# UbiquitousLearning/Mandheling-DSP-Training

Hardware: AMD Instinct MI355X
Metric: training images/sec + int8 MFMA TOPS, VGG-11 batch 256, 1/2/4/8 MI355X (higher is better)
Workload: dtype int8; 1 GPU; VGG11 NITI int8 training step (fwd+relu+pool, loss grad, weight grad, input grad, SGD), 3x32x32; global_batch=256, per_gpu_batch=256, parallelism=single GPU, streams=one stream (weight gradient, then input gradient, per layer)

## Files before the change

### include/niti_hip.h

```cpp
#ifndef NITI_HIP_H
#define NITI_HIP_H

#include <stddef.h>
#include <stdint.h>

#ifdef __cplusplus
extern "C" {
#endif

enum niti_error_code {
    NITI_NO_ERROR = 0,
    NITI_OUT_OF_MEMORY = 1,
    NITI_NOT_SUPPORT = 2,
    NITI_COMPUTE_SIZE_ERROR = 3,
    NITI_NO_EXECUTION = 4,
    NITI_INVALID_VALUE = 5,
    NITI_INPUT_DATA_ERROR = 10,
    NITI_CALL_BACK_STOP = 11
};

enum niti_op_type {
    NITI_OP_CONV_INT8 = 700,
    NITI_OP_DECONV_INT8 = 701,
    NITI_OP_RELU_INT8 = 703,
// ... 158 lines not shown
    int8_t* pool3_out;
    int8_t* pool3_arg;
    int relu, pool_relu, pool_h, pool_w;
    int zero_cls, zc_h, zc_w;
    int pool3_h, pool3_w, pool3_oh, pool3_ow;
} niti_requant_fused;
int niti_requant_act_fused(const int32_t* acc, int64_t rows, int ldc, const uint32_t* amax,
                           const niti_requant_fused* f, void* stream);
int niti_requant_grad(const int32_t* acc, int64_t n, const uint32_t* amax, int rule, int8_t* g_out,
                      int8_t* w_update, void* stream);
int niti_sgd_update(const int32_t* acc, const uint32_t* amax, int rule, int co, int ci, int kk, int cip, int cop,
                    int8_t* w_ohwi16, int8_t* wt_ihwo16, int8_t* g_out, void* stream);
int niti_sgd_update_wf(const int32_t* acc, const uint32_t* amax, int rule, int co, int ci, int kk, int cip, int cop,
                       int8_t* w_ohwi16, int8_t* wt_ihwo16, int8_t* g_out, int8_t* wf, int8_t* wft, void* stream);
typedef struct niti_sgd_combine_job {
    const int32_t* slab;
    int splits;
    int64_t stride;
    int64_t n;
    int32_t* acc;
    uint32_t* amax;
} niti_sgd_combine_job;
int niti_sgd_combine(const niti_sgd_combine_job* jobs, int n_jobs, void* stream);
int niti_nhwc16_to_chwn16(const int8_t* in, int n, int hw, int cp, int np, int8_t* out, void* stream);
int niti_ohwi16_to_ihwo16(const int8_t* w, int co, int ci, int kk, int cip, int cop, int8_t* wt, void* stream);
int niti_nchw_to_nhwc16(const int8_t* x, int n, int c, int hw, int cp, int8_t* out, void* stream);
int niti_nchw_to_chwn16(const int8_t* x, int n, int c, int hw, int cp, int np, int8_t* out, void* stream);
int niti_nhwc16_to_nchw(const int8_t* x, int n, int c, int hw, int cp, int8_t* out, void* stream);
int niti_oihw_to_ohwi16(const int8_t* w, int co, int ci, int kk, int cip, int8_t* out, void* stream);
int niti_ohwi16_to_oihw(const int8_t* w, int co, int ci, int kk, int cip, int8_t* out, void* stream);
int niti_residual_add(const int8_t* a, const int8_t* ea, const int8_t* b, const int8_t* eb, int64_t n, int32_t* z,
                      int8_t* ez, uint32_t* amax, void* stream);
int niti_residual_requant(const int8_t* a, const int8_t* ea, const int8_t* b, const int8_t* eb, int64_t n,
                          const uint32_t* amax, int8_t* ez, int8_t* exp_out, int relu, int8_t* out, void* stream);
int niti_residual_requant_relu_grad(const int8_t* a, const int8_t* ea, const int8_t* b, const int8_t* eb, int64_t n,
                                    const uint32_t* amax, int8_t* ez, int8_t* exp_out, const int8_t* relu_mask,
                                    int8_t* out, void* stream);
int niti_sum_pool(const int8_t* x, int n, int hw, int cp, int32_t* acc, uint32_t* amax, void* stream);
int niti_sum_pool_grad(const int8_t* dy, int n, int hw, int cp, int8_t* dx, void* stream);
int niti_im2col(const niti_geom* g, const int8_t* x, int kp, int8_t* xcol, void* stream);
int niti_im2col_nchw(const niti_geom* g, const int8_t* x_nchw, int kp, int8_t* xcol, void* stream);
int niti_maxpool(const int8_t* x, int n, int h, int w, int cp, int k, int s, int p, int8_t* y, int oh, int ow,
                 void* stream);
int niti_maxpool_grad(const int8_t* x, const int8_t* y, const int8_t* dy, int n, int h, int w, int cp, int k,
                      int s, int p, int oh, int ow, int relu, int8_t* dx, void* stream);
int niti_maxpool_grad_ws(const int8_t* x, const int8_t* y, const int8_t* dy, int n, int h, int w, int cp, int k,
// ... 113 lines not shown
```

### mandheling-dsp-training_amd/csrc/niti_capi.hip

```cpp
#include "../../include/niti_hip.h"
#include <memory>
#include <vector>

#include "niti_internal.hpp"
#include "niti_kernels.hpp"

struct niti_execution {
    niti::Execution* impl = nullptr;
    int op = 0;
    std::vector<void*> stage;
    std::vector<size_t> stage_bytes;
    uint32_t* err_host = nullptr;
    ~niti_execution() {
        delete impl;
        for (void* p : stage)
            if (p) (void)hipFree(p);
        if (err_host) (void)hipHostFree(err_host);
    }
};

namespace {
int code(hipError_t e) {
    if (e == hipSuccess) return NITI_NO_ERROR;
    if (e == hipErrorOutOfMemory) return NITI_OUT_OF_MEMORY;
// ... 588 lines not shown
    j.wft = wft;
    return code(niti::sgd_update_many(&j, 1, S(stream)));
}

int niti_sgd_combine(const niti_sgd_combine_job* jobs, int n_jobs, void* stream) {
    if (!jobs || n_jobs < 1 || n_jobs > niti::SGD_MAX_JOBS) return NITI_INVALID_VALUE;
    niti::SgdJob r[niti::SGD_MAX_JOBS];
    for (int j = 0; j < n_jobs; ++j) {
        const niti_sgd_combine_job& s = jobs[j];
        if (!s.slab || !s.acc || !s.amax || s.splits < 1 || s.n < 4 || s.n % 4 || s.stride % 4 || s.stride < s.n)
            return NITI_INVALID_VALUE;
        if (((uintptr_t)s.slab | (uintptr_t)s.acc) & 15) return NITI_INVALID_VALUE;
        r[j] = niti::SgdJob{};
        r[j].acc = s.acc;
        r[j].amax = s.amax;
        r[j].slab = s.slab;
        r[j].splits = s.splits;
        r[j].slab_stride = s.stride;
        r[j].slab_n = s.n;
    }
    return code(niti::sgd_combine_many(r, n_jobs, S(stream)));
}

int niti_nhwc16_to_chwn16(const int8_t* in, int n, int hw, int cp, int np, int8_t* out, void* stream) {
    return code(niti::nhwc16_to_chwn16(in, n, hw, cp, np, out, S(stream)));
}
int niti_ohwi16_to_ihwo16(const int8_t* w, int co, int ci, int kk, int cip, int cop, int8_t* wt, void* stream) {
    return code(niti::ohwi16_to_ihwo16(w, co, ci, kk, cip, cop, wt, S(stream)));
}
int niti_nchw_to_nhwc16(const int8_t* x, int n, int c, int hw, int cp, int8_t* out, void* stream) {
    return code(niti::nchw_to_nhwc16(x, n, c, hw, cp, out, S(stream)));
}
int niti_nchw_to_chwn16(const int8_t* x, int n, int c, int hw, int cp, int np, int8_t* out, void* stream) {
    return code(niti::nchw_to_chwn16(x, n, c, hw, cp, np, out, S(stream)));
}
int niti_nhwc16_to_nchw(const int8_t* x, int n, int c, int hw, int cp, int8_t* out, void* stream) {
    return code(niti::nhwc16_to_nchw(x, n, c, hw, cp, out, S(stream)));
}
int niti_oihw_to_ohwi16(const int8_t* w, int co, int ci, int kk, int cip, int8_t* out, void* stream) {
    return code(niti::oihw_to_ohwi16(w, co, ci, kk, cip, out, S(stream)));
}
int niti_ohwi16_to_oihw(const int8_t* w, int co, int ci, int kk, int cip, int8_t* out, void* stream) {
    return code(niti::ohwi16_to_oihw(w, co, ci, kk, cip, out, S(stream)));
}
int niti_residual_add(const int8_t* a, const int8_t* ea, const int8_t* b, const int8_t* eb, int64_t n, int32_t* z,
                      int8_t* ez, uint32_t* amax, void* stream) {
// ... 207 lines not shown
```

### mandheling-dsp-training_amd/csrc/niti_device.hpp

```cpp
#pragma once

#include <hip/hip_runtime.h>
#include <stdint.h>

#include "niti_kernels.hpp"

namespace niti {

typedef int v2i __attribute__((ext_vector_type(2)));
typedef int v4i __attribute__((ext_vector_type(4)));
typedef int v16i __attribute__((ext_vector_type(16)));
typedef signed char v16c __attribute__((ext_vector_type(16)));

constexpr uint32_t OOB = 0x80000000u;

__device__ __forceinline__ __amdgpu_buffer_rsrc_t make_rsrc(const void* p, uint32_t bytes) {
    return __builtin_amdgcn_make_buffer_rsrc((void*)p, (short)0, (int)bytes, 0x00020000);
}
__device__ __forceinline__ v4i buf_load16(__amdgpu_buffer_rsrc_t r, uint32_t off) {
    return __builtin_bit_cast(v4i, __builtin_amdgcn_raw_buffer_load_b128(r, (int)off, 0, 0));
}

struct FastDiv {
    uint32_t m = 1, s = 0, d = 1;
};
static inline FastDiv make_fastdiv(uint32_t d) {
    FastDiv f;
    f.d = d;
    f.s = 0;
    while ((1ull << f.s) < d) ++f.s;
    f.m = (uint32_t)((((uint64_t)1 << 32) * ((1ull << f.s) - d)) / d + 1);
    return f;
}
__device__ __forceinline__ uint32_t fdiv(const FastDiv& f, uint32_t n) { return (__umulhi(n, f.m) + n) >> f.s; }

__device__ __forceinline__ uint32_t uabs32(int v) { return v < 0 ? 0u - (uint32_t)v : (uint32_t)v; }

__device__ __forceinline__ uint32_t wave_max(uint32_t v) {
#pragma unroll
    for (int o = 32; o > 0; o >>= 1) {
        const uint32_t t = __shfl_xor(v, o, 64);
        v = v > t ? v : t;
    }
// ... 276 lines not shown
```

### mandheling-dsp-training_amd/csrc/niti_kernels.hip

```cpp
#include <stdlib.h>

#include <map>
#include <atomic>
#include <mutex>
#include <type_traits>
#include <vector>
#include <algorithm>
#include <stdio.h>

#include <hip/hip_ext.h>

#include "niti_device.hpp"
#include "niti_gridbar.hpp"
#include "niti_kernels.hpp"
#include "niti_sgd.hpp"
#include "niti_map.hpp"

namespace niti {


bool ConvGeom::finalize() {
    if (n <= 0 || c_in <= 0 || h <= 0 || w <= 0 || c_out <= 0 || kh <= 0 || kw <= 0) return false;
    if (sh <= 0 || sw <= 0 || dh <= 0 || dw <= 0) return false;
    const int keh = dh * (kh - 1) + 1, kew = dw * (kw - 1) + 1;
// ... 3188 lines not shown
    int64_t blocks = (n16 + 255) / 256;
    blocks = blocks < 1 ? 1 : blocks > 2048 ? 2048 : blocks;
    static const int pk = getenv("NITI_RES_PK") ? atoi(getenv("NITI_RES_PK")) : 1;
    hipLaunchKernelGGL(residual_requant_kernel, dim3((unsigned)blocks), dim3(256), 0, st, a, ea, b, eb, n16, amax, ez,
                       exp_out, relu, relu_mask, out, spec, slot, pk);
    return hipGetLastError();
}

struct Conv0 {
    const int8_t* x;
    const int8_t* w;
    uint32_t wbytes;
    int co, cop, oh, ow;
    int64_t units;
    uint32_t* amax;
    int8_t* out;
    int8_t* pool_out;
    int8_t* pool_c32;
    int8_t* out_c32;
    int8_t* pool_code;
    const int8_t *exp_in, *wscale;
    int8_t* exp_out;
    int relu;
};

template <int PASS>
__global__ void __launch_bounds__(256) conv0_kernel(Conv0 g) {
    const int lane = threadIdx.x & 63;
    const int wave = blockIdx.x * 4 + (threadIdx.x >> 6), nwaves = gridDim.x * 4;
    const int h = lane >> 5, c = lane & 31;
    const __amdgpu_buffer_rsrc_t rw = make_rsrc(g.w, g.wbytes);
    int s = 2, shift = 0;
    bool raw = false;
    if (PASS == 1) {
        const int bw = bitwidth_of(read_max(g.amax));
        shift = bw - 7;
        s = shift > 1 ? shift : 2;
        raw = shift <= 0;
        if (blockIdx.x == 0 && threadIdx.x == 0 && g.exp_out != nullptr) {
            const int inc = shift > 1 ? shift : (shift == 1 ? 2 : 0);
            *g.exp_out = (int8_t)((g.exp_in ? (int)*g.exp_in : 0) + (g.wscale ? (int)*g.wscale : 0) + inc);
        }
    }
    const int tiles = g.cop / 32;
    uint32_t m = 0;
    const int segs = g.ow / 32, pairs = g.oh / 2;
    for (int64_t u = wave; u < g.units; u += nwaves) {
        const int seg = (int)(u % segs);
        const int64_t rest = u / segs;
        const int pr = (int)(rest % pairs);
        const int64_t img = rest / pairs;
        const int64_t p0 = (img * g.oh + 2 * pr) * g.ow + seg * 32;
        v4i a[2];
#pragma unroll
        for (int r = 0; r < 2; ++r) a[r] = *(const v4i*)(g.x + (p0 + (int64_t)r * g.ow + c) * 32 + 16 * h);
        for (int t = 0; t < tiles; ++t) {
            const v4i b = buf_load16(rw, (uint32_t)((t * 32 + c) * 32 + 16 * h));
            v16i acc[2];
// ... 69 lines not shown
                        }
                    }
                    if ((c & 1) == 0) {
                        const int64_t pp = (img * (g.oh / 2) + pr) * (g.ow / 2) + seg * 16 + (c >> 1);
                        *(v4i*)(g.pool_out + pp * g.cop + t * 32 + 16 * h) = v;
                        if (g.pool_code != nullptr) *(v4i*)(g.pool_code + pp * g.cop + t * 32 + 16 * h) = code;
                        if (g.pool_c32 != nullptr) {
                            const int64_t hw2 = (int64_t)(g.oh / 2) * (g.ow / 2);
                            *(v4i*)(g.pool_c32 + ((img * tiles + t) * hw2 + pp - img * hw2) * 32 + 16 * h) = v;
                        }
                    }
                }
            }
        }
    }
    if (PASS == 0) {
        m = wave_max(m);
        __shared__ uint32_t red[4];
        if (lane == 0) red[threadIdx.x >> 6] = m;
        __syncthreads();
        if (threadIdx.x == 0) publish_max(g.amax, max(max(red[0], red[1]), max(red[2], red[3])));
    }
}

bool conv0_ok(const ConvGeom& g) {
    return g.kh == 1 && g.kw == 1 && g.c_in == 32 && g.cip == 32 && g.ow % 32 == 0 && g.oh % 2 == 0 && g.sh == 1 &&
           g.pt == 0 && g.cop % 32 == 0;
}

hipError_t conv0_fwd(const ConvGeom& g, const int8_t* xcol, const int8_t* w, uint32_t* amax, const ActOut& o,
                     int pass, hipStream_t st, int8_t* pool_c32, int8_t* out_c32, int8_t* pool_code) {
    if (!conv0_ok(g) || o.relu_mask != nullptr) return hipErrorInvalidValue;
    if (o.out == nullptr && (pass == 1 && (o.pool.pool_out == nullptr || pool_code == nullptr))) return hipErrorInvalidValue;
    if ((pool_c32 != nullptr || pool_code != nullptr) && o.pool.pool_out == nullptr) return hipErrorInvalidValue;
    Conv0 k{};
    k.x = xcol;
    k.w = w;
    k.wbytes = (uint32_t)((int64_t)g.c_out * 32);
    k.co = g.c_out;
    k.cop = g.cop;
    k.oh = g.oh;
    k.ow = g.ow;
    k.units = (int64_t)g.n * (g.oh / 2) * (g.ow / 32);
    k.amax = amax;
    k.out = o.out;
    k.pool_out = o.pool.pool_out;
    k.pool_c32 = pool_c32;
    k.out_c32 = out_c32;
    k.pool_code = pool_code;
    k.exp_in = o.exp_in;
    k.wscale = o.wscale;
    k.exp_out = o.exp_out;
    k.relu = o.relu;
    int64_t blocks = (k.units + 3) / 4;
    blocks = blocks > 1024 ? 1024 : blocks;
    if (pass == 0)
        hipLaunchKernelGGL(conv0_kernel<0>, dim3((unsigned)blocks), dim3(256), 0, st, k);
    else
        hipLaunchKernelGGL(conv0_kernel<1>, dim3((unsigned)blocks), dim3(256), 0, st, k);
    return hipGetLastError();
}

constexpr int RQ3_ROWS = 4;
struct Rq3Geom {
    FastDiv fq, fow, fch;
    int qpr, H, W, OH, rows;
    uint32_t units;
    int remap;
};
__device__ __forceinline__ void pool3_take(uint32_t o, int k, uint32_t& m, uint32_t& a) {
#pragma unroll
    for (int e = 0; e < 4; ++e) {
        const int ov = (int8_t)(o >> (8 * e)), mv = (int8_t)(m >> (8 * e)), av = (int8_t)(a >> (8 * e));
        if (av < 0 || ov > mv) {
            m = (m & ~(0xffu << (8 * e))) | (o & (0xffu << (8 * e)));
            a = (a & ~(0xffu << (8 * e))) | ((uint32_t)k << (8 * e));
        }
    }
}
__device__ __forceinline__ uint32_t rq4_relu(v4i v, int s) {
    const int h = s >> 1, odd = s & 1;
    uint32_t o = 0;
// ... 1109 lines not shown
```

### mandheling-dsp-training_amd/csrc/niti_kernels.hpp

```cpp
#pragma once

#include <hip/hip_runtime.h>
#include <stdint.h>
#include <stdlib.h>

#include "../../include/niti_hip.h"

namespace niti {

inline int round_up(int x, int m) { return (x + m - 1) / m * m; }

constexpr int MAX_SLOTS = 64;
constexpr int MAX_SLOT_STRIDE = 32;
constexpr int MAX_WORDS = MAX_SLOTS * MAX_SLOT_STRIDE;
constexpr size_t MAX_BYTES = MAX_WORDS * sizeof(uint32_t);

struct ConvGeom {
    int n, c_in, h, w;
    int c_out, kh, kw;
    int sh, sw, pt, pl, pb, pr, dh, dw;
    int oh, ow;
    int cip, cop, np;
    bool finalize();
};
// ... 125 lines not shown
};
struct Pool3 {
    int8_t* out = nullptr;
    int8_t* arg = nullptr;
    int H = 0, W = 0, OH = 0, OW = 0;
};
struct ActOut {
    int8_t* out = nullptr;
    int relu = 0;
    const int8_t* relu_mask = nullptr;
    const int8_t* exp_in = nullptr;
    const int8_t* wscale = nullptr;
    int8_t* exp_out = nullptr;
    PoolFuse pool;
    int8_t* out_p16 = nullptr;
    int zero_cls = 0, zc_h = 0, zc_w = 0;
    Pool3 pool3;
};
bool conv_fwd_phase2_separate(const ConvGeom& g, size_t ws_bytes);
bool conv0_ok(const ConvGeom& g);
hipError_t conv0_fwd(const ConvGeom& g, const int8_t* xcol, const int8_t* w, uint32_t* amax, const ActOut& o,
                     int pass, hipStream_t st,
                     int8_t* pool_c32 = nullptr, int8_t* out_c32 = nullptr, int8_t* pool_code = nullptr);
bool conv_dgrad_phase2_separate(const ConvGeom& g, size_t ws_bytes);
constexpr int GEMM_SPEC_SLOT_WORDS = 32;
constexpr int GEMM_SPEC_ALT_PAIRS = 8;
inline bool tune_spec() {
    static const bool on = getenv("NITI_TUNE_SPEC") && atoi(getenv("NITI_TUNE_SPEC")) == 1;
    return on;
}
bool conv_fwd_spec_ok(const ConvGeom& g);
bool conv_dgrad_spec_ok(const ConvGeom& g);
void gemm_speculate_bias(int bias);
size_t conv_fwd_spec_alt_bytes(const ConvGeom& g);
size_t conv_dgrad_spec_alt_bytes(const ConvGeom& g);
hipError_t conv_fwd_spec(const ConvGeom& g, const int8_t* x, const int8_t* w, uint32_t* amax, const ActOut& o,
                         uint32_t* slot, int pass, hipStream_t st, int8_t* alt = nullptr);
hipError_t conv_dgrad_spec(const ConvGeom& g, const int8_t* dy, const int8_t* wt, uint32_t* amax, const ActOut& o,
                           uint32_t* slot, int pass, hipStream_t st, int8_t* alt = nullptr);
struct FusedBar {
    uint32_t* bar = nullptr;
    uint32_t epoch = 0;
    uint32_t* err = nullptr;
    uint32_t spin_limit = 0;
};
unsigned long long gemm_fused_launches();
// ... 255 lines not shown
```

### mandheling-dsp-training_amd/csrc/niti_sgd.hpp

```cpp
#pragma once

#include "niti_device.hpp"
#include "niti_kernels.hpp"

#ifndef NITI_SGD_NT
#define NITI_SGD_NT 0
#endif
#ifndef NITI_SGD_PREFETCH
#define NITI_SGD_PREFETCH 0
#endif

namespace niti {

__device__ __forceinline__ int bitwidth_of(uint32_t m) { return m <= 1u ? 0 : 32 - __clz((int)(m - 1u)); }

__device__ __forceinline__ int32_t clip127(int32_t a) { return a > 127 ? 127 : (a < -127 ? -127 : a); }

__device__ __forceinline__ int32_t pow2_x86(int s) { return (int32_t)(1u << ((unsigned)s & 31u)); }

__device__ __forceinline__ int32_t psto_fast(int32_t a, int s) {
    const uint32_t ua = a < 0 ? 0u - (uint32_t)a : (uint32_t)a;
    const uint32_t q = ua >> s;
    const uint32_t prob = ua & ((1u << s) - 1u);
    const int h = s >> 1;
// ... 19 lines not shown

__device__ __forceinline__ int32_t psto_any(int32_t a, int s) {
    return (s >= 0 && s <= 30) ? psto_fast(a, s) : psto_generic(a, s);
}

struct SgdTileIn {
    v4i a[4];
    v16c w;
};
__device__ __forceinline__ void sgd_tile_load(const SgdJob& J, int ci0, int co0, int k, SgdTileIn& in) {
    const int t = threadIdx.x;
    const int r = t >> 2, c = (t & 3) * 16;
    if (co0 + r < J.co && ci0 + c < J.cip) {
        const int64_t idx = ((int64_t)(co0 + r) * J.kk + k) * J.cip + ci0 + c;
        const v4i* a4 = (const v4i*)(J.acc + idx);
#pragma unroll
        for (int q = 0; q < 4; ++q) in.a[q] = NITI_SGD_NT ? __builtin_nontemporal_load(a4 + q) : a4[q];
        in.w = *(const v16c*)(J.w + idx);
    }
}
__device__ __forceinline__ void sgd_tile_finish(const SgdJob& J, int bw, int ci0, int co0, int k, const SgdTileIn& in,
                                                int8_t (*T)[64 + 4]) {
    const int t = threadIdx.x;
    const int sh = bw - J.rule;
    {
        const int r = t >> 2, c = (t & 3) * 16;
        v16c wn;
#pragma unroll
        for (int j = 0; j < 16; ++j) wn[j] = 0;
        if (co0 + r < J.co && ci0 + c < J.cip) {
            const int64_t idx = ((int64_t)(co0 + r) * J.kk + k) * J.cip + ci0 + c;
            v16c g;
#pragma unroll
            for (int q = 0; q < 4; ++q) {
                const v4i v = in.a[q];
#pragma unroll
                for (int e = 0; e < 4; ++e) g[q * 4 + e] = (signed char)(bw == 0 ? 0 : psto_any(v[e], sh));
            }
#pragma unroll
            for (int j = 0; j < 16; ++j) wn[j] = (signed char)clip127((int32_t)in.w[j] - (int32_t)g[j]);
            *(v16c*)(J.w + idx) = wn;
            if (J.g_out != nullptr) *(v16c*)(J.g_out + idx) = g;
            if (J.wf != nullptr) {
                const int o = co0 + r, i0 = ci0 + c, cb = (J.ci + 31) / 32;
                *(v16c*)(J.wf + (((((int64_t)(o >> 5) * cb + (i0 >> 5)) * 9 + k) * 2 + ((i0 >> 4) & 1)) * 32 + (o & 31)) * 16) = wn;
            }
        }
#pragma unroll
        for (int j = 0; j < 16; ++j) T[r][c + j] = wn[j];
    }
    __syncthreads();
    if (J.wT != nullptr || J.wft != nullptr || J.subw != nullptr) {
        const int r = t >> 2, c = (t & 3) * 16;
        if (ci0 + r < J.ci && co0 + c < J.cop) {
            v16c o;
#pragma unroll
            for (int j = 0; j < 16; ++j) o[j] = T[c + j][r];
            if (J.wT != nullptr) *(v16c*)(J.wT + ((int64_t)(ci0 + r) * J.kk + k) * J.cop + co0 + c) = o;
            if (J.subw != nullptr) {
                const int ky = k / J.sub_kw, kx = k - ky * J.sub_kw;
// ... 141 lines not shown
```

### mandheling-dsp-training_amd/niti_amd/_lib.py

```python
from __future__ import annotations

import ctypes as C
import os
import re

_HERE = os.path.dirname(os.path.abspath(__file__))
LIB_PATH = os.environ.get("NITI_HIP_LIB") or os.path.join(_HERE, "_lib", "libniti_hip.so")
HEADER = os.path.join(os.path.dirname(os.path.dirname(_HERE)), "include", "niti_hip.h")

ERROR_NAMES = {0: "NO_ERROR", 1: "OUT_OF_MEMORY", 2: "NOT_SUPPORT", 3: "COMPUTE_SIZE_ERROR",
               4: "NO_EXECUTION", 5: "INVALID_VALUE", 10: "INPUT_DATA_ERROR", 11: "CALL_BACK_STOP"}
NOT_SUPPORT, INVALID_VALUE = 2, 5

OP_CONV_INT8 = 700
OP_DECONV_INT8 = 701
OP_RELU_INT8 = 703
OP_RELUGRAD_INT8 = 704
OP_MAXPOOL_INT8 = 705
OP_POOLGRAD_INT8 = 706
OP_LOSS_INT8 = 710
OP_LOSS_GRAD_INT8 = 711
OP_MATMUL_INT8 = 713
OP_PAD_INT8 = 714
OP_LEFTPOOLGRAD_INT8 = 718
# ... 33 lines not shown


class ConvCommon(C.Structure):
    _fields_ = [("kernel_x", C.c_int), ("kernel_y", C.c_int), ("stride_x", C.c_int), ("stride_y", C.c_int),
                ("dilate_x", C.c_int), ("dilate_y", C.c_int), ("pad_x", C.c_int), ("pad_y", C.c_int),
                ("has_pads", C.c_int), ("pads", C.c_int * 4), ("pad_mode", C.c_int),
                ("input_count", C.c_int), ("output_count", C.c_int), ("group", C.c_int)]


class Geom(C.Structure):
    _fields_ = [(n, C.c_int) for n in (
        "n", "c_in", "h", "w", "c_out", "kh", "kw", "stride_h", "stride_w", "pad_t", "pad_l", "pad_b",
        "pad_r", "dilate_h", "dilate_w", "oh", "ow", "cip", "cop", "np")]


class WgradP16Job(C.Structure):
    _fields_ = [("g", Geom), ("x_p16", C.c_void_p), ("dy_p16", C.c_void_p), ("acc", C.c_void_p),
                ("amax", C.c_void_p)]


class SgdCombineJob(C.Structure):
    _fields_ = [("slab", C.c_void_p), ("splits", C.c_int), ("stride", C.c_int64), ("n", C.c_int64),
                ("acc", C.c_void_p), ("amax", C.c_void_p)]


class ChainLayer(C.Structure):
    _fields_ = [(n, C.c_int) for n in ("c_out", "kernel", "stride", "pad", "relu", "pool", "flatten")]


class EvalTotals(C.Structure):
    _fields_ = [("images", C.c_uint64), ("top1", C.c_uint64), ("topk", C.c_uint64), ("loss_sum", C.c_double)]


class RequantFused(C.Structure):
    _fields_ = ([(n, C.c_void_p) for n in (
        "exp_in", "wscale", "exp_out", "relu_mask", "out_nhwc16", "pool_out", "pool_x", "pool_y", "pool_dx",
        "pool_dx_c32", "out_p16", "pool3_out", "pool3_arg")] + [(n, C.c_int) for n in (
            "relu", "pool_relu", "pool_h", "pool_w", "zero_cls", "zc_h", "zc_w", "pool3_h", "pool3_w", "pool3_oh",
            "pool3_ow")])


_lib = None


def header_functions():
    src = open(HEADER).read()
# ... 42 lines not shown
        "niti_nhwc16_to_c32": (ci, [vp, ci, ci, ci, ci, vp, vp]),
        "niti_weights_to_wf": (ci, [vp, ci, ci, ci, ci, vp, vp]),
        "niti_conv_fwd_rows": (ci, [C.POINTER(Geom), vp, vp, vp, vp, vp, ci, vp, vp, vp, ci, vp, vp, C.c_uint32, vp,
                                    vp]),
        "niti_conv_dgrad_rows": (ci, [C.POINTER(Geom), vp, vp, vp, vp, vp, ci, vp, vp, vp, vp, vp, vp, ci, vp, vp, C.c_uint32, vp, vp]),
        "niti_rows_spec_slot": (vp, [vp, ci]),
        "niti_conv_fwd_phase2": (ci, [C.POINTER(Geom), vp, vp, vp, vp, vp, vp, vp, ci, vp, vp, C.c_size_t, vp]),
        "niti_conv_dgrad_phase1": (ci, [C.POINTER(Geom), vp, vp, vp, vp, vp, C.c_size_t, vp]),
        "niti_conv_dgrad_phase2": (ci, [C.POINTER(Geom), vp, vp, vp, vp, vp, vp, vp, ci, vp, vp, C.c_size_t, vp]),
        "niti_nhwc16_to_p16": (ci, [vp, i64, ci, vp, vp]),
        "niti_diag_wgrad_stamps": (None, [vp]),
        "niti_diag_rowconv_stamps": (None, [vp]),
        "niti_conv_wgrad_p16_workspace": (ci, [C.POINTER(Geom), ci, C.POINTER(C.c_size_t)]),
        "niti_conv_wgrad_p16_acc": (ci, [C.POINTER(Geom), vp, vp, vp, vp, vp, C.c_size_t, ci, vp]),
        "niti_conv_wgrad_p16_many_workspace": (ci, [C.POINTER(WgradP16Job), ci, ci, ci, C.POINTER(C.c_size_t)]),
        "niti_conv_wgrad_p16_many": (ci, [C.POINTER(WgradP16Job), ci, ci, ci, vp, C.c_size_t, C.POINTER(ci), vp]),
        "niti_matmul_acc": (ci, [ci, ci, ci, vp, i64, vp, i64, vp, i64, vp, vp, C.c_size_t, vp]),
        "niti_absmax_i32": (ci, [vp, i64, vp, vp]),
        "niti_requant_act": (ci, [vp, i64, ci, vp, vp, vp, vp, ci, vp, vp, vp]),
        "niti_requant_act_fused": (ci, [vp, i64, ci, vp, C.POINTER(RequantFused), vp]),
        "niti_requant_grad": (ci, [vp, i64, vp, ci, vp, vp, vp]),
        "niti_sgd_update": (ci, [vp, vp, ci, ci, ci, ci, ci, ci, vp, vp, vp, vp]),
        "niti_sgd_combine": (ci, [C.POINTER(SgdCombineJob), ci, vp]),
        "niti_nhwc16_to_chwn16": (ci, [vp, ci, ci, ci, ci, vp, vp]),
        "niti_ohwi16_to_ihwo16": (ci, [vp, ci, ci, ci, ci, ci, vp, vp]),
        "niti_nchw_to_nhwc16": (ci, [vp, ci, ci, ci, ci, vp, vp]),
        "niti_nchw_to_chwn16": (ci, [vp, ci, ci, ci, ci, ci, vp, vp]),
        "niti_nhwc16_to_nchw": (ci, [vp, ci, ci, ci, ci, vp, vp]),
        "niti_oihw_to_ohwi16": (ci, [vp, ci, ci, ci, ci, vp, vp]),
        "niti_ohwi16_to_oihw": (ci, [vp, ci, ci, ci, ci, vp, vp]),
        "niti_residual_add": (ci, [vp, vp, vp, vp, i64, vp, vp, vp, vp]),
        "niti_residual_requant": (ci, [vp, vp, vp, vp, i64, vp, vp, vp, ci, vp, vp]),
        "niti_residual_requant_relu_grad": (ci, [vp, vp, vp, vp, i64, vp, vp, vp, vp, vp, vp]),
        "niti_sum_pool": (ci, [vp, ci, ci, ci, vp, vp, vp]),
        "niti_sum_pool_grad": (ci, [vp, ci, ci, ci, vp, vp]),
        "niti_im2col": (ci, [C.POINTER(Geom), vp, ci, vp, vp]),
        "niti_im2col_nchw": (ci, [C.POINTER(Geom), vp, ci, vp, vp]),
        "niti_sgd_update_wf": (ci, [vp, vp, ci, ci, ci, ci, ci, ci, vp, vp, vp, vp, vp, vp]),
        "niti_conv_rows_nhwc_ok": (ci, [C.POINTER(Geom), ci]),
        "niti_conv_plan_set": (ci, [C.POINTER(Geom), ci, vp]),
        "niti_maxpool": (ci, [vp] + [ci] * 7 + [vp, ci, ci, vp]),
        "niti_maxpool_grad": (ci, [vp, vp, vp] + [ci] * 10 + [vp, vp]),
        "niti_maxpool_grad_ws": (ci, [vp, vp, vp] + [ci] * 10 + [vp, vp, vp]),
        "niti_maxpool_arg": (ci, [vp] + [ci] * 7 + [vp, ci, ci, vp, vp]),
        "niti_maxpool_grad_arg": (ci, [vp, vp, vp] + [ci] * 10 + [vp, vp, vp]),
        "niti_relu_grad": (ci, [vp, vp, i64, vp, vp]),
# ... 76 lines not shown
```

### mandheling-dsp-training_amd/niti_amd/ops.py

```python
from __future__ import annotations

import ctypes as C

import torch

from . import _lib as L
from ._lib import check


def _stream(stream=None):
    if stream is not None:
        return stream
    return C.c_void_p(torch.cuda.current_stream().cuda_stream)


def _ptr(t):
    return None if t is None else C.c_void_p(t.data_ptr())


def tensor(t: torch.Tensor, dims, fmt=L.FORMAT_NCHW) -> L.Tensor:
    d = list(dims) + [1] * (4 - len(dims))
    v = L.Tensor(t.data_ptr(), (C.c_int * 4)(*d), fmt)
    v._keep = t
    return v
# ... 410 lines not shown
    if wT is None:
        wT = torch.zeros((ci, kh, kw, cop), dtype=torch.int8, device=acc.device)
    if g is None:
        g = torch.empty(acc.shape, dtype=torch.int8, device=acc.device)
    assert wT.shape == (ci, kh, kw, cop) and g.shape == acc.shape
    if wf is not None or wft is not None:
        check(L.lib().niti_sgd_update_wf(_ptr(acc), _ptr(amax), rule, co, ci, kh * kw, cip, cop, _ptr(w16), _ptr(wT),
                                         _ptr(g), _ptr(wf), _ptr(wft), _stream(stream)), "sgd_update_wf")
        return wT, g
    check(L.lib().niti_sgd_update(_ptr(acc), _ptr(amax), rule, co, ci, kh * kw, cip, cop, _ptr(w16), _ptr(wT), _ptr(g),
                                  _stream(stream)), "sgd_update")
    return wT, g


def sgd_combine(jobs, stream=None):
    arr = (L.SgdCombineJob * len(jobs))()
    for j, (slab, n, acc, amax) in enumerate(jobs):
        assert slab.dtype == torch.int32 and slab.dim() == 2 and slab.is_contiguous() and acc.numel() >= n
        arr[j].slab, arr[j].splits, arr[j].stride, arr[j].n = slab.data_ptr(), slab.shape[0], slab.shape[1], n
        arr[j].acc, arr[j].amax = acc.data_ptr(), amax.data_ptr()
    check(L.lib().niti_sgd_combine(arr, len(jobs), _stream(stream)), "sgd_combine")


def residual_add(a, ea, b, eb, amax, stream=None, ez=None):
    assert a.shape == b.shape and a.dtype == b.dtype == torch.int8
    z = torch.empty(a.shape, dtype=torch.int32, device=a.device)
    if ez is None:
        ez = torch.zeros(1, dtype=torch.int8, device=a.device)
    check(L.lib().niti_residual_add(_ptr(a), _ptr(ea), _ptr(b), _ptr(eb), a.numel(), _ptr(z), _ptr(ez), _ptr(amax),
                                    _stream(stream)), "residual_add")
    return z, ez


def residual_range(a, ea, b, eb, amax, stream=None):
    assert a.shape == b.shape and a.dtype == b.dtype == torch.int8
    check(L.lib().niti_residual_add(_ptr(a), _ptr(ea), _ptr(b), _ptr(eb), a.numel(), None, None, _ptr(amax),
                                    _stream(stream)), "residual_range")


def residual_requant(a, ea, b, eb, amax, ez=None, exp_out=None, relu=False, relu_mask=None, stream=None):
    assert a.shape == b.shape and a.dtype == b.dtype == torch.int8
    out = torch.empty(a.shape, dtype=torch.int8, device=a.device)
    if ez is None:
        ez = torch.zeros(1, dtype=torch.int8, device=a.device)
    if exp_out is None:
        exp_out = torch.zeros(1, dtype=torch.int8, device=a.device)
# ... 152 lines not shown
```

Before: 760,200 images/s.

## Add persistent buffer-resource conv0 kernel and expose batched SGD and conv0 APIs

Adds a new conv0 forward kernel, specialised on the number of 32-channel output tiles. It keeps weights in registers, prefetches the next unit's input, uses buffer loads and stores with fast division, and picks a requant rule at compile time. The grid is sized to resident workgroups instead of a fixed cap, and the old kernel is kept as a fallback for wide outputs. The SGD tile finish now uses readfirstlane-uniform shifts with a fast path. C and Python bindings are added for batched SGD, input im2col and conv0. Risks include added register pressure and a new code path that only runs if callers use it.

Measured after the change: 771,100 images/s (median of 6 runs). 1.4% higher.

```diff
diff --git a/include/niti_hip.h b/include/niti_hip.h
--- a/include/niti_hip.h
+++ b/include/niti_hip.h
@@ -204,6 +204,34 @@
     uint32_t* amax;
 } niti_sgd_combine_job;
 int niti_sgd_combine(const niti_sgd_combine_job* jobs, int n_jobs, void* stream);
+typedef struct niti_sgd_job {
+    const int32_t* acc;
+    const uint32_t* amax;
+    int rule, co, ci, kk, cip, cop;
+    int8_t* w_ohwi16;
+    int8_t* wt_ihwo16;
+    int8_t* g_out;
+    int8_t* wf;
+    int8_t* wft;
+} niti_sgd_job;
+int niti_sgd_update_many(const niti_sgd_job* jobs, int n_jobs, void* stream);
+int niti_input_im2col(const void* in, int quant, int n, int c, int h, int w, int kh, int kw, int pad_t, int pad_l,
+                      const uint64_t* stats, int64_t count, int8_t* x_nchw, int8_t* xcol, int8_t* ascale,
+                      const int8_t* w0, int co0, int cop0, uint32_t* amax0, void* stream);
+typedef struct niti_conv0_out {
+    int8_t* out;
+    int8_t* pool_out;
+    int8_t* pool_code;
+    int8_t* pool_c32;
+    int8_t* out_c32;
+    const int8_t* exp_in;
+    const int8_t* wscale;
+    int8_t* exp_out;
+    int relu;
+} niti_conv0_out;
+int niti_conv0_fwd(const niti_geom* g, const int8_t* xcol, const int8_t* w, uint32_t* amax, const niti_conv0_out* o,
+                   int pass, void* stream);
+void niti_diag_conv0_blocks(int n);
 int niti_nhwc16_to_chwn16(const int8_t* in, int n, int hw, int cp, int np, int8_t* out, void* stream);
 int niti_ohwi16_to_ihwo16(const int8_t* w, int co, int ci, int kk, int cip, int cop, int8_t* wt, void* stream);
 int niti_nchw_to_nhwc16(const int8_t* x, int n, int c, int hw, int cp, int8_t* out, void* stream);
diff --git a/mandheling-dsp-training_amd/csrc/niti_capi.hip b/mandheling-dsp-training_amd/csrc/niti_capi.hip
--- a/mandheling-dsp-training_amd/csrc/niti_capi.hip
+++ b/mandheling-dsp-training_amd/csrc/niti_capi.hip
@@ -634,6 +634,56 @@
     return code(niti::sgd_combine_many(r, n_jobs, S(stream)));
 }
 
+int niti_sgd_update_many(const niti_sgd_job* jobs, int n_jobs, void* stream) {
+    if (!jobs || n_jobs < 1 || n_jobs > niti::SGD_MAX_JOBS) return NITI_INVALID_VALUE;
+    niti::SgdJob r[niti::SGD_MAX_JOBS];
+    for (int j = 0; j < n_jobs; ++j) {
+        const niti_sgd_job& s = jobs[j];
+        if (!s.acc || !s.amax || !s.w_ohwi16 || (s.rule != 2 && s.rule != 3)) return NITI_INVALID_VALUE;
+        if (s.co < 1 || s.ci < 1 || s.kk < 1 || s.cip < s.ci || s.cop < s.co || s.cip % 16 || s.cop % 16)
+            return NITI_INVALID_VALUE;
+        if ((s.wf || s.wft) && (s.kk != 9 || s.ci % 32 != 0 || s.co % 32 != 0)) return NITI_NOT_SUPPORT;
+        r[j] = niti::SgdJob{s.acc, s.amax, s.rule, s.co, s.ci, s.kk, s.cip, s.cop, s.w_ohwi16, s.wt_ihwo16, s.g_out};
+        r[j].wf = s.wf;
+        r[j].wft = s.wft;
+    }
+    return code(niti::sgd_update_many(r, n_jobs, S(stream)));
+}
+
+int niti_input_im2col(const void* in, int quant, int n, int c, int h, int w, int kh, int kw, int pad_t, int pad_l,
+                      const uint64_t* stats, int64_t count, int8_t* x_nchw, int8_t* xcol, int8_t* ascale,
+                      const int8_t* w0, int co0, int cop0, uint32_t* amax0, void* stream) {
+    if (!in || !xcol || n <= 0 || h <= 0 || w <= 0 || pad_t < 0 || pad_l < 0) return NITI_INVALID_VALUE;
+    if (!niti::input_im2col_ok(c, kh, kw)) return NITI_NOT_SUPPORT;
+    if (quant && (!stats || count <= 0)) return NITI_INVALID_VALUE;
+    niti::Conv0Range r0;
+    if (w0 != nullptr) {
+        r0.w = w0;
+        r0.co = co0;
+        r0.cop = cop0;
+        r0.amax = amax0;
+    }
+    return code(niti::input_im2col(in, quant != 0, n, c, h, w, kh, kw, pad_t, pad_l,
+                                   (const unsigned long long*)stats, quant ? 1 : 0, count, x_nchw, xcol, ascale,
+                                   S(stream), r0));
+}
+
+int niti_conv0_fwd(const niti_geom* g, const int8_t* xcol, const int8_t* w, uint32_t* amax, const niti_conv0_out* o,
+                   int pass, void* stream) {
+    niti::ConvGeom r;
+    if (!g || !xcol || !w || !amax || !o || pass < 0 || pass > 1 || !to_geom(g, &r)) return NITI_INVALID_VALUE;
+    if (!niti::conv0_ok(r)) return NITI_NOT_SUPPORT;
+    niti::ActOut a;
+    a.out = o->out;
+    a.relu = o->relu;
+    a.exp_in = o->exp_in;
+    a.wscale = o->wscale;
+    a.exp_out = o->exp_out;
+    a.pool.pool_out = o->pool_out;
+    return code(niti::conv0_fwd(r, xcol, w, amax, a, pass, S(stream), o->pool_c32, o->out_c32, o->pool_code));
+}
+void niti_diag_conv0_blocks(int n) { niti::diag_conv0_blocks(n); }
+
 int niti_nhwc16_to_chwn16(const int8_t* in, int n, int hw, int cp, int np, int8_t* out, void* stream) {
     return code(niti::nhwc16_to_chwn16(in, n, hw, cp, np, out, S(stream)));
 }
diff --git a/mandheling-dsp-training_amd/csrc/niti_device.hpp b/mandheling-dsp-training_amd/csrc/niti_device.hpp
--- a/mandheling-dsp-training_amd/csrc/niti_device.hpp
+++ b/mandheling-dsp-training_amd/csrc/niti_device.hpp
@@ -19,6 +19,11 @@
 }
 __device__ __forceinline__ v4i buf_load16(__amdgpu_buffer_rsrc_t r, uint32_t off) {
     return __builtin_bit_cast(v4i, __builtin_amdgcn_raw_buffer_load_b128(r, (int)off, 0, 0));
+}
+
+__device__ __forceinline__ void buf_store16(__amdgpu_buffer_rsrc_t r, uint32_t off, v4i v) {
+    typedef unsigned int v4u __attribute__((ext_vector_type(4)));
+    __builtin_amdgcn_raw_buffer_store_b128(__builtin_bit_cast(v4u, v), r, (int)off, 0, 0);
 }
 
 struct FastDiv {
diff --git a/mandheling-dsp-training_amd/csrc/niti_kernels.hip b/mandheling-dsp-training_amd/csrc/niti_kernels.hip
--- a/mandheling-dsp-training_amd/csrc/niti_kernels.hip
+++ b/mandheling-dsp-training_amd/csrc/niti_kernels.hip
@@ -3234,10 +3234,12 @@
     const int8_t *exp_in, *wscale;
     int8_t* exp_out;
     int relu;
+    uint32_t xbytes, obytes, pbytes;
+    FastDiv fseg, fpair;
 };
 
 template <int PASS>
-__global__ void __launch_bounds__(256) conv0_kernel(Conv0 g) {
+__global__ void __launch_bounds__(256) conv0_wide_kernel(Conv0 g) {
     const int lane = threadIdx.x & 63;
     const int wave = blockIdx.x * 4 + (threadIdx.x >> 6), nwaves = gridDim.x * 4;
     const int h = lane >> 5, c = lane & 31;
@@ -3245,7 +3247,7 @@
     int s = 2, shift = 0;
     bool raw = false;
     if (PASS == 1) {
-        const int bw = bitwidth_of(read_max(g.amax));
+        const int bw = __builtin_amdgcn_readfirstlane(bitwidth_of(read_max(g.amax)));
         shift = bw - 7;
         s = shift > 1 ? shift : 2;
         raw = shift <= 0;
@@ -3361,6 +3363,148 @@
         if (threadIdx.x == 0) publish_max(g.amax, max(max(red[0], red[1]), max(red[2], red[3])));
     }
 }
+
+template <int PASS, int NT>
+__global__ void __launch_bounds__(256) conv0_kernel(Conv0 g) {
+    const int lane = threadIdx.x & 63;
+    const uint32_t wave = (uint32_t)__builtin_amdgcn_readfirstlane((int)(blockIdx.x * 4 + (threadIdx.x >> 6)));
+    const uint32_t nwaves = gridDim.x * 4, units = (uint32_t)g.units;
+    const int h = lane >> 5, c = lane & 31;
+    const __amdgpu_buffer_rsrc_t rw = make_rsrc(g.w, g.wbytes), rx = make_rsrc(g.x, g.xbytes);
+    const __amdgpu_buffer_rsrc_t ro = make_rsrc(g.out, g.obytes), rc = make_rsrc(g.out_c32, g.obytes);
+    const __amdgpu_buffer_rsrc_t rp = make_rsrc(g.pool_out, g.pbytes), rpc = make_rsrc(g.pool_c32, g.pbytes);
+    const __amdgpu_buffer_rsrc_t rpk = make_rsrc(g.pool_code, g.pbytes);
+    const uint32_t segs = g.fseg.d, pairs = g.fpair.d, ow = (uint32_t)g.ow, oh = (uint32_t)g.oh, cop = NT * 32u;
+    uint32_t gm = 0;
+    if (PASS == 1) gm = g.amax[lane * MAX_SLOT_STRIDE];
+    v4i wa[NT];
+#pragma unroll
+    for (int t = 0; t < NT; ++t) wa[t] = buf_load16(rw, (uint32_t)((t * 32 + c) * 32 + 16 * h));
+    const uint32_t lx = (uint32_t)(c * 32 + 16 * h);
+    auto xload = [&](uint32_t u, v4i(&a)[2]) {
+        const uint32_t q = fdiv(g.fseg, u), seg = u - q * segs;
+        const uint32_t o = u < units ? (2u * q * ow + seg * 32u) * 32u + lx : OOB;
+        a[0] = buf_load16(rx, o);
+        a[1] = buf_load16(rx, o + ow * 32u);
+    };
+    v4i a[2];
+    xload(wave, a);
+    int s = 2, cls = 0, lo = -128;
+    if (PASS == 1) {
+        const int shift = __builtin_amdgcn_readfirstlane(bitwidth_of(wave_max(gm))) - 7;
+        s = shift > 1 ? shift : 2;
+        cls = shift <= 0 ? 0 : (g.relu ? 1 : 2);
+        lo = g.relu ? 0 : -128;
+        if (blockIdx.x == 0 && threadIdx.x == 0 && g.exp_out != nullptr) {
+            const int inc = shift > 1 ? shift : (shift == 1 ? 2 : 0);
+            *g.exp_out = (int8_t)((g.exp_in ? (int)*g.exp_in : 0) + (g.wscale ? (int)*g.wscale : 0) + inc);
+        }
+    }
+    uint32_t m = 0;
+    auto pack = [&](const int32_t* v) {
+        uint32_t d[4];
+#pragma unroll
+        for (int j = 0; j < 4; ++j) {
+            const uint32_t p01 = __builtin_amdgcn_perm((uint32_t)v[4 * j + 1], (uint32_t)v[4 * j], 0x0c0c0400u);
+            const uint32_t p23 = __builtin_amdgcn_perm((uint32_t)v[4 * j + 3], (uint32_t)v[4 * j + 2], 0x0c0c0400u);
+            d[j] = __builtin_amdgcn_perm(p23, p01, 0x05040100u);
+        }
+        const auto x02 = __builtin_amdgcn_permlane32_swap(d[0], d[2], false, false);
+        const auto x13 = __builtin_amdgcn_permlane32_swap(d[1], d[3], false, false);
+        return v4i{(int)x02[0], (int)x02[1], (int)x13[0], (int)x13[1]};
+    };
+    auto run = [&](auto rule) {
+        constexpr int RULE = decltype(rule)::value;
+        const uint32_t hh = (uint32_t)s >> 1, hs = (uint32_t)s - hh, odd = (uint32_t)s & 1u;
+        auto rq = [&](int32_t v) -> int32_t {
+            if constexpr (RULE == 0) {
+                return max((int32_t)(int8_t)v, lo);
+            } else {
+                const uint32_t x = RULE == 1 ? (uint32_t)max(v, 0) : uabs32(v);
+                const uint32_t qp = __builtin_amdgcn_ubfe(x, hh, hs), pr = __builtin_amdgcn_ubfe(x, 0, hh) << odd;
+                const int32_t r = (int32_t)min((x >> s) + (qp > pr ? 1u : 0u), 127u);
+                return RULE == 1 ? r : (v < 0 ? -r : r);
+            }
+        };
+        for (uint32_t u = wave; u < units; u += nwaves) {
+            v4i an[2];
+            xload(u + nwaves, an);
+            const uint32_t q = fdiv(g.fseg, u), seg = u - q * segs;
+            const uint32_t img = fdiv(g.fpair, q), pr = q - img * pairs;
+            const uint32_t p0 = 2u * q * ow + seg * 32u;
+            const uint32_t pp = q * (ow / 2) + seg * 16u + (c >> 1);
+#pragma unroll
+            for (int t = 0; t < NT; ++t) {
+                v16i acc[2];
+#pragma unroll
+                for (int r = 0; r < 2; ++r)
+                    acc[r] = __builtin_amdgcn_mfma_i32_32x32x32_i8(wa[t], a[r], v16i{}, 0, 0, 0);
+                if (PASS == 0) {
+#pragma unroll
+                    for (int r = 0; r < 2; ++r)
+#pragma unroll
+                        for (int i = 0; i < 16; ++i) m = max(m, uabs32(acc[r][i]));
+                    continue;
+                }
+                int32_t v[2][16];
+                v4i qv[2];
+#pragma unroll
+                for (int r = 0; r < 2; ++r) {
+#pragma unroll
+                    for (int i = 0; i < 16; ++i) v[r][i] = rq(acc[r][i]);
+                    qv[r] = pack(v[r]);
+                    if (g.out != nullptr) buf_store16(ro, (p0 + r * ow + c) * cop + t * 32 + 16 * h, qv[r]);
+                    if (g.out_c32 != nullptr)
+                        buf_store16(rc, (((img * NT + t) * oh + 2 * pr + r) * ow + seg * 32u + c) * 32u + 16 * h, qv[r]);
+                }
+                if (g.pool_out != nullptr) {
+                    int32_t pm[16];
+#pragma unroll
+                    for (int i = 0; i < 16; ++i) {
+                        const int v0 = max(v[0][i], v[1][i]);
+                        pm[i] = max(v0, __builtin_amdgcn_mov_dpp(v0, 0xB1, 0xF, 0xF, false));
+                    }
+                    const v4i pv = pack(pm);
+                    v4i code{0, 0, 0, 0};
+                    if (g.pool_code != nullptr) {
+#pragma unroll
+                        for (int k = 0; k < 4; ++k) {
+                            const uint32_t t1 = (uint32_t)__builtin_amdgcn_mov_dpp(qv[0][k], 0xB1, 0xF, 0xF, false);
+                            const uint32_t t3 = (uint32_t)__builtin_amdgcn_mov_dpp(qv[1][k], 0xB1, 0xF, 0xF, false);
+                            code[k] = (int)pool_code4((uint32_t)qv[0][k], t1, (uint32_t)qv[1][k], t3, (uint32_t)pv[k],
+                                                      g.relu != 0);
+                        }
+                    }
+                    if ((c & 1) == 0) {
+                        const uint32_t po = pp * cop + t * 32 + 16 * h;
+                        buf_store16(rp, po, pv);
+                        if (g.pool_code != nullptr) buf_store16(rpk, po, code);
+                        if (g.pool_c32 != nullptr)
+                            buf_store16(rpc, (((img * NT + t) * pairs + pr) * (ow / 2) + seg * 16u + (c >> 1)) * 32u + 16 * h, pv);
+                    }
+                }
+            }
+            a[0] = an[0];
+            a[1] = an[1];
+        }
+    };
+    if (PASS == 0 || cls == 0)
+        run(std::integral_constant<int, 0>{});
+    else if (cls == 1)
+        run(std::integral_constant<int, 1>{});
+    else
+        run(std::integral_constant<int, 2>{});
+    if (PASS == 0) {
+        m = wave_max(m);
+        __shared__ uint32_t red[4];
+        if (lane == 0) red[threadIdx.x >> 6] = m;
+        __syncthreads();
+        if (threadIdx.x == 0) publish_max(g.amax, max(max(red[0], red[1]), max(red[2], red[3])));
+    }
+}
+
+static std::atomic<int> g_conv0_blocks{0};
+void diag_conv0_blocks(int n) { g_conv0_blocks = n > 0 ? n : 0; }
 
 bool conv0_ok(const ConvGeom& g) {
     return g.kh == 1 && g.kw == 1 && g.c_in == 32 && g.cip == 32 && g.ow % 32 == 0 && g.oh % 2 == 0 && g.sh == 1 &&
@@ -3392,11 +3536,27 @@
     k.exp_out = o.exp_out;
     k.relu = o.relu;
     int64_t blocks = (k.units + 3) / 4;
-    blocks = blocks > 1024 ? 1024 : blocks;
-    if (pass == 0)
-        hipLaunchKernelGGL(conv0_kernel<0>, dim3((unsigned)blocks), dim3(256), 0, st, k);
-    else
-        hipLaunchKernelGGL(conv0_kernel<1>, dim3((unsigned)blocks), dim3(256), 0, st, k);
+    const int64_t pixels = (int64_t)g.n * g.oh * g.ow;
+    if (g.cop > 64 || pixels * 64 >= ((int64_t)1 << 31)) {
+        blocks = blocks > 1024 ? 1024 : blocks;
+        if (pass == 0)
+            hipLaunchKernelGGL(conv0_wide_kernel<0>, dim3((unsigned)blocks), dim3(256), 0, st, k);
+        else
+            hipLaunchKernelGGL(conv0_wide_kernel<1>, dim3((unsigned)blocks), dim3(256), 0, st, k);
+        return hipGetLastError();
+    }
+    k.xbytes = (uint32_t)(pixels * 32);
+    k.obytes = (uint32_t)(pixels * g.cop);
+    k.pbytes = (uint32_t)(pixels / 4 * g.cop);
+    k.fseg = make_fastdiv((uint32_t)(g.ow / 32));
+    k.fpair = make_fastdiv((uint32_t)(g.oh / 2));
+    using Kern = void (*)(Conv0);
+    const Kern f = pass == 0 ? (g.cop == 32 ? conv0_kernel<0, 1> : conv0_kernel<0, 2>)
+                             : (g.cop == 32 ? conv0_kernel<1, 1> : conv0_kernel<1, 2>);
+    const int forced = g_conv0_blocks.load();
+    const int res = forced > 0 ? forced : resident_wgs((const void*)f);
+    if (res > 0 && blocks > res) blocks = res;
+    hipLaunchKernelGGL(f, dim3((unsigned)blocks), dim3(256), 0, st, k);
     return hipGetLastError();
 }
 
diff --git a/mandheling-dsp-training_amd/csrc/niti_kernels.hpp b/mandheling-dsp-training_amd/csrc/niti_kernels.hpp
--- a/mandheling-dsp-training_amd/csrc/niti_kernels.hpp
+++ b/mandheling-dsp-training_amd/csrc/niti_kernels.hpp
@@ -171,6 +171,7 @@
 hipError_t conv0_fwd(const ConvGeom& g, const int8_t* xcol, const int8_t* w, uint32_t* amax, const ActOut& o,
                      int pass, hipStream_t st,
                      int8_t* pool_c32 = nullptr, int8_t* out_c32 = nullptr, int8_t* pool_code = nullptr);
+void diag_conv0_blocks(int n);
 bool conv_dgrad_phase2_separate(const ConvGeom& g, size_t ws_bytes);
 constexpr int GEMM_SPEC_SLOT_WORDS = 32;
 constexpr int GEMM_SPEC_ALT_PAIRS = 8;
diff --git a/mandheling-dsp-training_amd/csrc/niti_sgd.hpp b/mandheling-dsp-training_amd/csrc/niti_sgd.hpp
--- a/mandheling-dsp-training_amd/csrc/niti_sgd.hpp
+++ b/mandheling-dsp-training_amd/csrc/niti_sgd.hpp
@@ -65,7 +65,8 @@
 __device__ __forceinline__ void sgd_tile_finish(const SgdJob& J, int bw, int ci0, int co0, int k, const SgdTileIn& in,
                                                 int8_t (*T)[64 + 4]) {
     const int t = threadIdx.x;
-    const int sh = bw - J.rule;
+    const int ubw = __builtin_amdgcn_readfirstlane(bw);
+    const int sh = ubw - __builtin_amdgcn_readfirstlane(J.rule);
     {
         const int r = t >> 2, c = (t & 3) * 16;
         v16c wn;
@@ -74,11 +75,15 @@
         if (co0 + r < J.co && ci0 + c < J.cip) {
             const int64_t idx = ((int64_t)(co0 + r) * J.kk + k) * J.cip + ci0 + c;
             v16c g;
-#pragma unroll
-            for (int q = 0; q < 4; ++q) {
-                const v4i v = in.a[q];
-#pragma unroll
-                for (int e = 0; e < 4; ++e) g[q * 4 + e] = (signed char)(bw == 0 ? 0 : psto_any(v[e], sh));
+            if (ubw == 0) {
+#pragma unroll
+                for (int j = 0; j < 16; ++j) g[j] = 0;
+            } else if (sh >= 0 && sh <= 30) {
+#pragma unroll
+                for (int j = 0; j < 16; ++j) g[j] = (signed char)psto_fast(in.a[j >> 2][j & 3], sh);
+            } else {
+#pragma unroll
+                for (int j = 0; j < 16; ++j) g[j] = (signed char)psto_generic(in.a[j >> 2][j & 3], sh);
             }
 #pragma unroll
             for (int j = 0; j < 16; ++j) wn[j] = (signed char)clip127((int32_t)in.w[j] - (int32_t)g[j]);
diff --git a/mandheling-dsp-training_amd/niti_amd/_lib.py b/mandheling-dsp-training_amd/niti_amd/_lib.py
--- a/mandheling-dsp-training_amd/niti_amd/_lib.py
+++ b/mandheling-dsp-training_amd/niti_amd/_lib.py
@@ -79,6 +79,17 @@
 class SgdCombineJob(C.Structure):
     _fields_ = [("slab", C.c_void_p), ("splits", C.c_int), ("stride", C.c_int64), ("n", C.c_int64),
                 ("acc", C.c_void_p), ("amax", C.c_void_p)]
+
+
+class SgdJob(C.Structure):
+    _fields_ = ([("acc", C.c_void_p), ("amax", C.c_void_p)] +
+                [(n, C.c_int) for n in ("rule", "co", "ci", "kk", "cip", "cop")] +
+                [(n, C.c_void_p) for n in ("w_ohwi16", "wt_ihwo16", "g_out", "wf", "wft")])
+
+
+class Conv0Out(C.Structure):
+    _fields_ = ([(n, C.c_void_p) for n in ("out", "pool_out", "pool_code", "pool_c32", "out_c32", "exp_in",
+                                           "wscale", "exp_out")] + [("relu", C.c_int)])
 
 
 class ChainLayer(C.Structure):
@@ -167,6 +178,10 @@
         "niti_requant_grad": (ci, [vp, i64, vp, ci, vp, vp, vp]),
         "niti_sgd_update": (ci, [vp, vp, ci, ci, ci, ci, ci, ci, vp, vp, vp, vp]),
         "niti_sgd_combine": (ci, [C.POINTER(SgdCombineJob), ci, vp]),
+        "niti_sgd_update_many": (ci, [C.POINTER(SgdJob), ci, vp]),
+        "niti_input_im2col": (ci, [vp] + [ci] * 9 + [vp, i64, vp, vp, vp, vp, ci, ci, vp, vp]),
+        "niti_conv0_fwd": (ci, [C.POINTER(Geom), vp, vp, vp, C.POINTER(Conv0Out), ci, vp]),
+        "niti_diag_conv0_blocks": (None, [C.c_int]),
         "niti_nhwc16_to_chwn16": (ci, [vp, ci, ci, ci, ci, vp, vp]),
         "niti_ohwi16_to_ihwo16": (ci, [vp, ci, ci, ci, ci, ci, vp, vp]),
         "niti_nchw_to_nhwc16": (ci, [vp, ci, ci, ci, ci, vp, vp]),
diff --git a/mandheling-dsp-training_amd/niti_amd/ops.py b/mandheling-dsp-training_amd/niti_amd/ops.py
--- a/mandheling-dsp-training_amd/niti_amd/ops.py
+++ b/mandheling-dsp-training_amd/niti_amd/ops.py
@@ -456,6 +456,48 @@
     check(L.lib().niti_sgd_combine(arr, len(jobs), _stream(stream)), "sgd_combine")
 
 
+def sgd_update_many(jobs, stream=None):
+    arr = (L.SgdJob * len(jobs))()
+    for j, job in enumerate(jobs):
+        acc, w16 = job["acc"], job["w16"]
+        co, kh, kw, cip = acc.shape
+        assert acc.dtype == torch.int32 and w16.shape == acc.shape and acc.is_contiguous() and w16.is_contiguous()
+        arr[j].acc, arr[j].amax = acc.data_ptr(), job["amax"].data_ptr()
+        arr[j].rule, arr[j].co, arr[j].ci, arr[j].kk = job.get("rule", 2), co, job["ci"], kh * kw
+        arr[j].cip, arr[j].cop = cip, r16(co)
+        arr[j].w_ohwi16 = w16.data_ptr()
+        for name, key in (("wt_ihwo16", "wT"), ("g_out", "g"), ("wf", "wf"), ("wft", "wft")):
+            t = job.get(key)
+            setattr(arr[j], name, None if t is None else t.data_ptr())
+    check(L.lib().niti_sgd_update_many(arr, len(jobs), _stream(stream)), "sgd_update_many")
+
+
+def input_im2col(x, kernel, pad, stats=None, count=None, w0=None, co0=0, amax0=None, stream=None):
+    assert x.dim() == 4 and x.is_contiguous() and x.dtype in (torch.uint8, torch.int8)
+    quant = x.dtype == torch.uint8
+    assert not quant or stats is not None
+    n, c, h, w = x.shape
+    oh, ow = h + 2 * pad - kernel + 1, w + 2 * pad - kernel + 1
+    xcol = torch.empty((n * oh * ow, 32), dtype=torch.int8, device=x.device)
+    x8 = torch.empty(x.shape, dtype=torch.int8, device=x.device)
+    ascale = torch.zeros(1, dtype=torch.int8, device=x.device)
+    check(L.lib().niti_input_im2col(_ptr(x), 1 if quant else 0, n, c, h, w, kernel, kernel, pad, pad, _ptr(stats),
+                                    int(count or x.numel()), _ptr(x8), _ptr(xcol), _ptr(ascale), _ptr(w0), co0,
+                                    0 if w0 is None else w0.shape[0], _ptr(amax0), _stream(stream)), "input_im2col")
+    return xcol, x8, ascale
+
+
+def conv0_fwd(g, xcol, w, amax, pass_, *, out=None, pool_out=None, pool_code=None, pool_c32=None, out_c32=None,
+              exp_in=None, wscale=None, exp_out=None, relu=False, stream=None):
+    o = L.Conv0Out()
+    for name, t in (("out", out), ("pool_out", pool_out), ("pool_code", pool_code), ("pool_c32", pool_c32),
+                    ("out_c32", out_c32), ("exp_in", exp_in), ("wscale", wscale), ("exp_out", exp_out)):
+        setattr(o, name, None if t is None else t.data_ptr())
+    o.relu = 1 if relu else 0
+    check(L.lib().niti_conv0_fwd(C.byref(g), _ptr(xcol), _ptr(w), _ptr(amax), C.byref(o), pass_, _stream(stream)),
+          "conv0_fwd")
+
+
 def residual_add(a, ea, b, eb, amax, stream=None, ez=None):
     assert a.shape == b.shape and a.dtype == b.dtype == torch.int8
     z = torch.empty(a.shape, dtype=torch.int32, device=a.device)
```
